# GDMCF/GDMCF

Measured on AMD Instinct MI355X. Metric: training users/sec, higher is better.
Workload: dtype f32; 1 GPU; yelp-shape synthetic rows, batch=400/GPU, dims=[1000], T=5, noise_scale=0.01, linear-var, mean_type=x0, reweight, AdamW lr=1e-5 (BASELINE configs[1]); n_items=34395, global_batch=400, parallelism=dp1, batch_rows=device CSR rows (CsrBatch)

## Files before the change

### gdmcf_amd/build.py

```python
import concurrent.futures
import hashlib
import os
import re
import subprocess
import sys

CSRC = os.path.join(os.path.dirname(os.path.abspath(__file__)), "csrc")
SOURCES = ["capi.hip", "dp_exchange.hip", "gemm_f32.hip", "gemm_bf16.hip", "gemm_split.hip", "gemm_small.hip", "gemm_dr.hip", "gemm_dr_tn.hip", "gemm_dr_fat.hip", "gemm_dr_kn.hip", "prep_input.hip", "noise.hip", "loss_tail.hip", "adamw.hip", "rows.hip", "reduce.hip", "linear.hip", "topk_spmm.hip", "spmm_bundle.hip", "score_topk.hip", "bpr.hip", "cat.hip", "gather_fwd.hip", "ntxent.hip", "latent_step.hip"]
HEADERS = ["common.h", "draws.h", "gemm_dr.h", "gemm_epilogue.h", os.path.join("..", "..", "include", "gdmcf_hip.h")]
LIB = os.path.join(CSRC, "libgdmcf_hip.so")
ASM_LINT = ("gemm_dr_tn.hip", "gemm_split.hip")
STORE_LINT = ("gemm_f32.hip", "gemm_bf16.hip", "gemm_dr_fat.hip", "gemm_dr_kn.hip", "score_topk.hip", "latent_step.hip")
NO_SPILL = ("gemm_f32.hip", "gemm_bf16.hip", "gemm_split.hip", "gemm_dr_tn.hip", "score_topk.hip", "cat.hip", "gather_fwd.hip", "ntxent.hip", "latent_step.hip")
FLAGS = ["--offload-arch=gfx950", "-O3", "-std=c++17", "-fPIC", "-Wall", "-Wno-unused-function"]


def _hipcc():
    for c in (os.environ.get("HIPCC"), "/opt/rocm/bin/hipcc", "hipcc"):
        if c and (os.path.isabs(c) and os.path.exists(c) or not os.path.isabs(c)):
            return c
    raise RuntimeError("hipcc not found")


def _digest():
    h = hashlib.sha256()
    for f in SOURCES + HEADERS:
        with open(os.path.join(CSRC, f), "rb") as fh:
            h.update(fh.read())
    h.update(" ".join(FLAGS).encode())
    return h.hexdigest()


_REG = re.compile(r"\bv(\d+)\b|\bv\[(\d+):(\d+)\]")


def _regs(text):
    out = set()
    for m in _REG.finditer(text):
        if m.group(1) is not None:
            out.add(int(m.group(1)))
        else:
            out.update(range(int(m.group(2)), int(m.group(3)) + 1))
    return out


_SREG = re.compile(r"\bs(\d+)\b|\bs\[(\d+):(\d+)\]")


def _sregs(text):
    out = set()
    for m in _SREG.finditer(text):
        if m.group(1) is not None:
            out.add(int(m.group(1)))
        else:
            out.update(range(int(m.group(2)), int(m.group(3)) + 1))
    return out


def lint_ring_registers(asm_text, kernel_prefix="dr_tn_kernel"):
    bad, seen = [], 0
    for m in re.finditer(r"^(\S*%s\S*):[^\n]*\n(.*?)\n\s*s_endpgm" % kernel_prefix, asm_text, flags=re.S | re.M):
        name, body = m.group(1), m.group(2)
        seen += 1
        lines = [ln.split(";")[0].strip() for ln in body.splitlines()]
        lines = [ln for ln in lines if ln and not ln.endswith(":") and not ln.startswith(".")]
        ring = set()
# ... 107 lines not shown

        state = [None] * len(blocks)
        state[0] = {}
        work = [0]
        while work:
            bi = work.pop()
            out = transfer(bi, state[bi], False)
            for sj in succ[bi]:
                if state[sj] is None:
                    state[sj] = dict(out)
                    work.append(sj)
                else:
                    changed = False
                    for r, rk in out.items():
                        if state[sj].get(r, 65) > rk:
                            state[sj][r] = rk
                            changed = True
                    if changed:
                        work.append(sj)
        for bi in range(len(blocks)):
            if state[bi] is not None:
                transfer(bi, state[bi], True)
        bad += [f"{name}: {msg}" for msg, k in sorted(found.items(), key=lambda kv: kv[1])]
    if not nk:
        bad.append("no kernel with inline-asm loads in the assembly (lint out of date?)")
    return bad


def lint_store_data(asm_text):
    bad = []
    for m in re.finditer(r"^(_Z\S+):[^\n]*\n(.*?)\n\s*s_endpgm", asm_text, flags=re.S | re.M):
        name, body = m.group(1), m.group(2)
        lines = [ln.split(";")[0].strip() for ln in body.splitlines()]
        lines = [ln for ln in lines if ln and not ln.startswith(".") and not ln.endswith(":")]
        for k, ln in enumerate(lines):
            mnem, _, ops = ln.partition(" ")
            if not re.match(r"(buffer|global|flat|scratch)_store_dwordx[34]$", mnem):
                continue
            parts = [o.strip() for o in ops.split(",")]
            data = _regs(parts[1] if mnem.startswith(("global", "flat", "scratch")) else parts[0])
            left = 2
            for nxt in lines[k + 1:k + 8]:
                nm, _, nops = nxt.partition(" ")
                if nm == "s_nop":
                    left -= int(nops.strip() or 0) + 1
                else:
                    nparts = [o.strip() for o in nops.split(",")]
                    if nm.startswith("v_") and nparts and _regs(nparts[0]) & data and left > 0:
                        bad.append(f"{name}: data register of `{ln}` rewritten {2 - left} wait state(s) later by `{nxt}`")
                        break
                    left -= 1
                if left <= 0:
                    break
    return bad


def build(force=False, verbose=True):
    stamp = os.path.join(CSRC, ".build_stamp")
    dig = _digest()
    if not force and os.path.exists(LIB) and os.path.exists(stamp) and open(stamp).read() == dig:
        return LIB
    hipcc = _hipcc()
    objs = []

    def compile_one(src):
        obj = os.path.join(CSRC, src.replace(".hip", ".o"))
        cmd = [hipcc] + FLAGS + ["-c", os.path.join(CSRC, src), "-o", obj]
        guarded = src in NO_SPILL
        if guarded:
            cmd.append("-Rpass-analysis=kernel-resource-usage")
        r = subprocess.run(cmd, capture_output=True, text=True)
        if r.returncode != 0:
            raise RuntimeError(f"hipcc failed for {src}:\n{r.stderr}")
        err = r.stderr
        if guarded:
            name, bad = None, []
            for line in err.splitlines():
                if "Function Name:" in line:
                    name = line.split("Function Name:")[1].split()[0]
                elif "VGPRs Spill:" in line and int(line.split("VGPRs Spill:")[1].split()[0]) > 0:
                    bad.append(name)
            if bad:
                raise RuntimeError(f"{src}: register spills in {len(bad)} kernel(s) with uncounted asm loads, e.g. {bad[0]}")
            err = err if ("warning:" in err or "error:" in err) else ""
        if verbose and err.strip():
            print(err, file=sys.stderr)
        if src in ASM_LINT or src in STORE_LINT:
            asm = os.path.join(CSRC, src.replace(".hip", ".lint.s"))
            r2 = subprocess.run([hipcc] + FLAGS + ["-S", "--cuda-device-only", os.path.join(CSRC, src), "-o", asm],
                                capture_output=True, text=True)
            if r2.returncode != 0:
                raise RuntimeError(f"hipcc -S failed for {src}:\n{r2.stderr}")
            text = open(asm).read()
            os.remove(asm)
            bad = lint_store_data(text)
            if src in ASM_LINT:
                bad += lint_vmcnt(text)
            if src == "gemm_dr_tn.hip":
                bad += lint_ring_registers(text)
            if bad:
                raise RuntimeError(f"{src}: ISA lint failed (lint_store_data / lint_vmcnt / lint_ring_registers):\n  " + "\n  ".join(bad[:12]))
        return obj

    with concurrent.futures.ThreadPoolExecutor(max_workers=min(8, len(SOURCES))) as ex:
        objs = list(ex.map(compile_one, SOURCES))
    cmd = [hipcc, "--offload-arch=gfx950", "-shared", "-fPIC", "-o", LIB] + objs
    r = subprocess.run(cmd, capture_output=True, text=True)
    if r.returncode != 0:
        raise RuntimeError(f"link failed:\n{r.stderr}")
    with open(stamp, "w") as fh:
        fh.write(dig)
    if verbose:
        print(f"built {LIB}")
    return LIB


if __name__ == "__main__":
    build(force="--force" in sys.argv)
```

### gdmcf_amd/csrc/gemm_dr.h

```cpp
#pragma once

#include "common.h"

namespace {
struct DrArgs {
    GdGemm g;
    int tiles_m, tiles_n, m_fastest;
    int ksp;
    int ctr;
    const GdAdamHyper* adam_dev;
    int stagger;
};
}

struct DrRoutes {
    bool dw;
    bool adamw;
    bool kn;
    bool fat;
};
DrRoutes& dr_routes();
int dr_cu_count();
int dr_stagger();

int gd_dr_tn_launch(GdGemm& g, hipStream_t s);
int gd_dr_kn_launch(GdGemm& g, hipStream_t s);
int gd_dr_fat_launch(int epi, GdGemm& g, hipStream_t s);
```

### gdmcf_amd/csrc/gemm_dr.hip

```cpp
#include <stdlib.h>

#include "gemm_dr.h"

int dr_cu_count() {
    static int n_cu = 0;
    if (n_cu == 0) {
        int dev = 0;
        hipDeviceProp_t prop;
        n_cu = (hipGetDevice(&dev) == hipSuccess && hipGetDeviceProperties(&prop, dev) == hipSuccess) ? prop.multiProcessorCount : 256;
    }
    return n_cu;
}

static bool dr_env_on(const char* name) {
    const char* v = getenv(name);
    return v == nullptr || atoi(v) != 0;
}
DrRoutes& dr_routes() {
    static DrRoutes r = {dr_env_on("GDMCF_DR_DW"), dr_env_on("GDMCF_DR_ADAMW"), dr_env_on("GDMCF_DR_KN"), dr_env_on("GDMCF_DR_FAT")};
    return r;
}

int dr_stagger() {
    static const int stagger = getenv("GDMCF_DR_STAGGER") ? atoi(getenv("GDMCF_DR_STAGGER")) : 3;
    return stagger;
}

int gd_gemm_dr_launch(int layA, int layB, int epi, GdGemm& g, hipStream_t s) {
    if (g.bf16) return GD_DR_NOT_TAKEN;
    if (g.accumulate || g.C16 || (g.splits > 1 && epi != GD_EPI_SLAB)) return GD_DR_NOT_TAKEN;
    if (layA == GD_LAY_MC && layB == GD_LAY_MC) {
        if (epi == GD_EPI_ADAMW) return gd_gemm_dr_adamw_multi(&g, 1, s);
        if (epi == GD_EPI_STORE) return gd_dr_tn_launch(g, s);
    } else if (layA == GD_LAY_KC && layB == GD_LAY_MC) {
        if (epi == GD_EPI_SLAB) return gd_dr_kn_launch(g, s);
    } else if (layA == GD_LAY_KC && layB == GD_LAY_KC) {
        if (epi == GD_EPI_LOSS || epi == GD_EPI_POST) return gd_dr_fat_launch(epi, g, s);
    }
    return GD_DR_NOT_TAKEN;
}
```

### gdmcf_amd/csrc/linear.hip

```cpp
#include <stdlib.h>

#include "common.h"

int gd_splitk_reduce(const float* slabs, int64_t slab_stride, int splits, int64_t ld_slab, int M, int N, int mode,
                     const float* bias, const float* rowscale, const float* aact, int64_t ldact, int act, float* out,
                     int64_t ldo, hipStream_t s);
int gd_colsum(const float* dZ, int64_t ld, const float* rs, int M, int N, float* db, hipStream_t s);
int gd_rowpart_reduce(const float* rowpart, int ld, int M, int nt, float* rowsum, hipStream_t s);

namespace {

static const int TARGET_WGS = getenv("GDMCF_TARGET_WGS") ? atoi(getenv("GDMCF_TARGET_WGS")) : 760;

thread_local int t_gemm_prec = GDMCF_GEMM_F32;

int pick_class(int M, int N, bool fused, int prec) {
    if (prec == GDMCF_GEMM_BF16 && M > 128) {
        const long pad = (long)gd_cdiv(M, 208) * 208;
        const long tiles = (pad / 208) * gd_cdiv(N, 256);
        const long rounds = (tiles + 255) / 256;
        if (pad * 10 <= (long)M * 11 && pad / 208 <= 2 && (!fused || tiles * 100 >= rounds * 256 * 85)) return 3;
    }
    if (prec == GDMCF_GEMM_F32X3 && M > 128 && N >= 128) {
        const long pad = (long)gd_cdiv(M, 208) * 208;
// ... 84 lines not shown
    const int prev = t_gemm_prec;
    if (mode == GDMCF_GEMM_F32 || mode == GDMCF_GEMM_BF16 || mode == GDMCF_GEMM_F32X3) t_gemm_prec = mode;
    return prev;
}

size_t gdmcf_linear_ws_bytes(int M, int N, int K) {
    if (M <= 0 || N <= 0 || K <= 0) return 0;
    size_t need = 0;
    for (int prec = GDMCF_GEMM_F32; prec <= GDMCF_GEMM_F32X3; ++prec) {
        const int cf = pick_class(M, N, false, prec), cb = pick_class(M, K, false, prec);
        size_t f = (size_t)pick_splits(M, N, K, cf, prec) * M * round4(N);
        if (prec == GDMCF_GEMM_F32) {
            const size_t fk = (size_t)gd_dr_kn_splits(M, N, K) * M * round4(N);
            f = f > fk ? f : fk;
        }
        size_t b = (size_t)pick_splits(M, K, N, cb, prec) * M * round4(K);
        if (prec == GDMCF_GEMM_F32) {
            const size_t bk = (size_t)gd_dr_kn_splits(M, K, N) * M * round4(K);
            b = b > bk ? b : bk;
        }
        need = need > f ? need : f;
        need = need > b ? need : b;
    }
    return need * sizeof(float) + 256;
}

int gdmcf_loss_tiles(int N) { return gd_cdiv(N, 16); }

int gdmcf_linear_fwd_f32(const float* A, int64_t lda, const float* W, int64_t ldw, const float* bias, int act, int M,
                         int N, int K, float* C, int64_t ldc, void* ws, size_t ws_bytes, void* stream) {
    GD_CHECK_SHAPE(M > 0 && N > 0 && K > 0 && lda >= K && ldw >= K && ldc >= N, "linear_fwd: bad shape");
    GD_CHECK_ARG(act == 0 || act == 1, "linear_fwd: bad activation");
    hipStream_t s = (hipStream_t)stream;
    const int cls = pick_class(M, N, false, t_gemm_prec);
    const int splits = pick_splits(M, N, K, cls, t_gemm_prec);
    GdGemm g = {};
    g.bf16 = t_gemm_prec;
    g.A = A; g.lda = lda; g.B = W; g.ldb = ldw; g.M = M; g.N = N; g.K = K;
    g.m_fastest = gd_cdiv(M, gd_gemm_tile_m(cls)) <= gd_cdiv(N, gd_gemm_tile_n(cls));
    g.bias = bias; g.act = act; g.prof_tag = 1;
    if (splits == 1) {
        g.splits = 1; g.C = C; g.ldc = ldc;
        attach_result_shadow(g);
        attach_shadows(g, GD_LAY_KC, GD_LAY_KC);
        return gd_gemm_launch(GD_LAY_KC, GD_LAY_KC, GD_EPI_BIAS_ACT, cls, g, s);
    }
    const int64_t lds_ = round4(N);
    const size_t need = (size_t)splits * M * lds_ * sizeof(float);
    if (ws == nullptr || ws_bytes < need) {
        gdmcf_set_error("linear_fwd: workspace %zu < %zu bytes", ws_bytes, need);
        return GDMCF_E_WORKSPACE;
    }
    g.splits = splits; g.C = (float*)ws; g.ldc = lds_; g.slab_stride = (int64_t)M * lds_;
    attach_shadows(g, GD_LAY_KC, GD_LAY_KC);
    int rc = gd_gemm_launch(GD_LAY_KC, GD_LAY_KC, GD_EPI_SLAB, cls, g, s);
    if (rc) return rc;
    const int real_splits = gd_cdiv(K, g.kchunk);
    return gd_splitk_reduce((const float*)ws, g.slab_stride, real_splits, lds_, M, N, 0, bias, nullptr, nullptr, 0,
                            act, C, ldc, s);
}

int gdmcf_linear_fwd_wt_f32(const float* A, int64_t lda, const float* Wt, int64_t ldwt, const float* bias, int act, int M, int N,
                            int K, float* C, int64_t ldc, void* ws, size_t ws_bytes, void* stream) {
    GD_CHECK_SHAPE(M > 0 && N > 0 && K > 0 && lda >= K && ldwt >= N && ldc >= N, "linear_fwd_wt: bad shape");
    GD_CHECK_ARG(act == 0 || act == 1, "linear_fwd_wt: bad activation");
    if (t_gemm_prec != GDMCF_GEMM_F32) {
        gdmcf_set_error("linear_fwd_wt: float32 GEMM mode only (the bf16 / f32x3 modes keep the weight in its own orientation)");
        return GDMCF_E_UNSUPPORTED;
    }
    hipStream_t s = (hipStream_t)stream;
    const int cls = pick_class(M, N, false, t_gemm_prec);
    const int splits = pick_splits(M, N, K, cls, t_gemm_prec);
    const int64_t lds_ = round4(N);
    const size_t need = (size_t)splits * M * lds_ * sizeof(float);
    if (ws == nullptr || ws_bytes < need) {
        gdmcf_set_error("linear_fwd_wt: workspace %zu < %zu bytes", ws_bytes, need);
        return GDMCF_E_WORKSPACE;
    }
    GdGemm g = {};
    g.A = A; g.lda = lda; g.B = Wt; g.ldb = ldwt; g.M = M; g.N = N; g.K = K;
    g.m_fastest = gd_cdiv(M, gd_gemm_tile_m(cls)) <= gd_cdiv(N, gd_gemm_tile_n(cls));
    g.splits = splits; g.C = (float*)ws; g.ldc = lds_; g.slab_stride = (int64_t)M * lds_; g.prof_tag = 1;
    g.ws_cap = ws_bytes;
    int rc = gd_gemm_launch(GD_LAY_KC, GD_LAY_MC, GD_EPI_SLAB, cls, g, s);
    if (rc) return rc;
    const int real_splits = gd_cdiv(K, g.kchunk);
    return gd_splitk_reduce((const float*)ws, g.slab_stride, real_splits, lds_, M, N, 0, bias, nullptr, nullptr, 0, act, C, ldc, s);
}

int gdmcf_linear_loss_fwd_f32(const float* A, int64_t lda, const float* W, int64_t ldw, const float* bias,
                              const float* target, int64_t ldt, const float* alpha, int M, int N, int K, float* out,
                              int64_t ldo, float* diff, int64_t ldd, float* rowpart, float* rowsum, void* stream) {
    GD_CHECK_SHAPE(M > 0 && N > 0 && K > 0 && lda >= K && ldw >= K && ldt >= N && ldd >= N, "linear_loss_fwd: bad shape");
    GD_CHECK_SHAPE(out == nullptr || ldo >= N, "linear_loss_fwd: ldo < N");
    hipStream_t s = (hipStream_t)stream;
    const int cls = pick_class(M, N, true, t_gemm_prec);
    GdGemm g = {};
    g.bf16 = t_gemm_prec;
    g.A = A; g.lda = lda; g.B = W; g.ldb = ldw; g.M = M; g.N = N; g.K = K; g.splits = 1;
    g.m_fastest = gd_cdiv(M, gd_gemm_tile_m(cls)) <= gd_cdiv(N, gd_gemm_tile_n(cls));
    g.bias = bias; g.aux = target; g.ldaux = ldt; g.r0 = alpha; g.out2 = out; g.ldout2 = ldo;
    g.prof_tag = 2;
    g.C = diff; g.ldc = ldd; g.rowpart = rowpart; g.ld_rowpart = gdmcf_loss_tiles(N);
    attach_result_shadow(g);
    attach_shadows(g, GD_LAY_KC, GD_LAY_KC);
    int rc = gd_gemm_launch(GD_LAY_KC, GD_LAY_KC, GD_EPI_LOSS, cls, g, s);
// ... 150 lines not shown
```

### gdmcf_amd/csrc/gemm_dr_fat.hip

```cpp
#include <stdlib.h>

#include "gemm_dr.h"

namespace {

template <int NB, int EPI>
__global__ __launch_bounds__(256, 1) void dr_fat_kernel(const DrArgs d) {
    static_assert(EPI == GD_EPI_LOSS || EPI == GD_EPI_POST, "output layer with a fused epilogue");
    static_assert(NB >= 4 && NB <= 12, "5 x NB accumulator blocks must fit 256 registers");
    constexpr int TMB = 5;
    const GdGemm& g = d.g;
    const int lane = threadIdx.x & 63;
    const int wave = __builtin_amdgcn_readfirstlane(threadIdx.x >> 6);
    const int r = lane & 15, q = lane >> 4;
    extern __shared__ __attribute__((aligned(16))) float dr_lds[];
    float* const lds = dr_lds + wave * (2 * NB * 256);
    const int nblk = gridDim.x, per = nblk >> 3;
    const int wl = ((nblk & 7) == 0 ? ((int)(blockIdx.x & 7) * per + (int)(blockIdx.x >> 3)) : (int)blockIdx.x) * 4 + wave;
    const int n_waves = nblk * 4;
    const int ntiles = d.tiles_m * d.tiles_n;
    const __amdgpu_buffer_rsrc_t srdA = __builtin_amdgcn_make_buffer_rsrc(const_cast<float*>(g.A), 0, (int)(((int64_t)(g.M - 1) * g.lda + g.K) * 4), 0x00020000);
    const __amdgpu_buffer_rsrc_t srdB = __builtin_amdgcn_make_buffer_rsrc(const_cast<float*>(g.B), 0, (int)(((int64_t)(g.N - 1) * g.ldb + g.K) * 4), 0x00020000);
    const int NCH = d.ksp;
    const int c_mask = g.K >> 4;
    const int w_off = (lane >> 2) * 16 + (((lane & 3) ^ ((((lane >> 2) >> 2) & 1) << 1)) << 2);
    const int r_off = r * 16 + ((q ^ (((r >> 2) & 1) << 1)) << 2);
    for (int tile = wl; tile < ntiles; tile += n_waves) {
        const int tm = tile % d.tiles_m, tn = tile / d.tiles_m;
        const int m0 = tm * (16 * TMB), n0 = tn * (16 * NB);
        uint32_t offA[TMB], offB[NB];
#pragma unroll
        for (int i = 0; i < TMB; ++i) offA[i] = (uint32_t)((m0 + 16 * i + r) * g.lda + 4 * q) * 4u;
#pragma unroll
        for (int p = 0; p < NB; ++p) offB[p] = (uint32_t)(((int64_t)(n0 + 16 * p + (lane >> 2)) * g.ldb + 4 * (lane & 3)) * 4);
        f32x4 acc[TMB][NB];
#pragma unroll
        for (int i = 0; i < TMB; ++i)
#pragma unroll
            for (int b = 0; b < NB; ++b) acc[i][b] = f32x4{0.f, 0.f, 0.f, 0.f};
        f32x4 xa[2][TMB], G[NB], FB[NB];
#pragma unroll
        for (int i = 0; i < TMB; ++i) xa[0][i] = __builtin_bit_cast(f32x4, __builtin_amdgcn_raw_buffer_load_b128(srdA, offA[i], 0, 0));
#pragma unroll
        for (int p = 0; p < NB; ++p) G[p] = __builtin_bit_cast(f32x4, __builtin_amdgcn_raw_buffer_load_b128(srdB, offB[p], 0, 0));
#pragma unroll
        for (int p = 0; p < NB; ++p) *reinterpret_cast<f32x4*>(lds + p * 256 + w_off) = G[p];

#define GD_FAT_CHUNK(PAR, c)                                                                                          \
        {                                                                                                             \
             \
            const uint32_t kn = ((c) + 1 < NCH) ? (uint32_t)((c) + 1) * 64u : 0x80000000u;                            \
            _Pragma("unroll") for (int b = 0; b < NB; ++b)                                                            \
                FB[b] = *reinterpret_cast<const f32x4*>(lds + (PAR) * (NB * 256) + b * 256 + r_off);                  \
            if ((c) >= c_mask) {  \
                 \
                _Pragma("unroll") for (int e = 0; e < 4; ++e) {                                                       \
                    const bool keep = (c) * 16 + 4 * q + e < g.K;                                                     \
                    _Pragma("unroll") for (int i = 0; i < TMB; ++i) xa[PAR][i][e] = keep ? xa[PAR][i][e] : 0.f;       \
                    _Pragma("unroll") for (int b = 0; b < NB; ++b) FB[b][e] = keep ? FB[b][e] : 0.f;                  \
                }                                                                                                     \
            }                                                                                                         \
            __builtin_amdgcn_sched_barrier(0);                                                                        \
            _Pragma("unroll") for (int sx = 0; sx < 4; ++sx) {                                                        \
                _Pragma("unroll") for (int n = 0; n < TMB * NB; ++n) {                                                \
                    const int i = n / NB, b = n % NB;                                                                 \
                    if (sx == 0 && i == 0) asm volatile("" : "+v"(FB[b]));  \
                    if (sx == 0 && b == 0) asm volatile("" : "+v"(xa[PAR][i]));                                       \
                    acc[i][b] = __builtin_amdgcn_mfma_f32_16x16x4f32(xa[PAR][i][sx], FB[b][sx], acc[i][b], 0, 0, 0);  \
                     \
                    if (sx < 2 && n % 5 == 2) {      \
                        const int l = (sx == 0) ? n / 5 : NB + n / 5;                                                 \
                        if (l < TMB + NB) {                                                                           \
                            __builtin_amdgcn_sched_barrier(0);                                                        \
                            if (l < TMB)                                                                              \
                                xa[(PAR) ^ 1][l] = __builtin_bit_cast(f32x4, __builtin_amdgcn_raw_buffer_load_b128(   \
                                    srdA, offA[l], kn, 0));                                                           \
                            else                                                                                      \
                                G[l - TMB] = __builtin_bit_cast(f32x4, __builtin_amdgcn_raw_buffer_load_b128(         \
                                    srdB, offB[l - TMB], kn, 0));                                                     \
                            __builtin_amdgcn_sched_barrier(0);                                                        \
                        }                                                                                             \
                    }                                                                                                 \
                    if (sx == 3 && n % 4 == 1 && n / 4 < NB) {   \
                        __builtin_amdgcn_sched_barrier(0);                                                            \
                        *reinterpret_cast<f32x4*>(lds + ((PAR) ^ 1) * (NB * 256) + (n / 4) * 256 + w_off) = G[n / 4]; \
                        __builtin_amdgcn_sched_barrier(0);                                                            \
                    }                                                                                                 \
                }                                                                                                     \
                __builtin_amdgcn_sched_barrier(0);                                                                    \
            }                                                                                                         \
        }
        const int c_pf = d.stagger > 0 ? ((NCH > d.stagger + 2 ? NCH - d.stagger : 0) & ~1) : -2;
        for (int c = 0; c + 1 < NCH; c += 2) {
            if constexpr (EPI == GD_EPI_POST) {
                if (c == c_pf) {
                    typedef __attribute__((address_space(3))) void* lds_vp;
                    constexpr int NJL = (16 * NB * 4 + 127) / 128 + 1;
                    constexpr int NPI = (80 * NJL + 63) / 64;
                    float* const scratch = dr_lds + 4 * (2 * NB * 256) + wave * 64;
                    const __amdgpu_buffer_rsrc_t srdX = __builtin_amdgcn_make_buffer_rsrc(
                        const_cast<float*>(g.aux), 0, (int)(((int64_t)(g.M - 1) * g.ldaux + g.N) * 4), 0x00020000);
#pragma unroll
                    for (int pi = 0; pi < NPI; ++pi) {
                        const int t = min(pi * 64 + lane, 80 * NJL - 1);
                        const int row = min(m0 + t % 80, g.M - 1), j = t / 80;
                        const int col = min(j < NJL - 1 ? n0 + 32 * j : n0 + 16 * NB - 1, g.N - 1);
                        __builtin_amdgcn_raw_ptr_buffer_load_lds(srdX, (lds_vp)scratch, 4, (int)(((int64_t)row * g.ldaux + col) * 4), 0, 0, 0);
                    }
                }
            }
            GD_FAT_CHUNK(0, c);
            GD_FAT_CHUNK(1, c + 1);
        }
        if (NCH & 1) GD_FAT_CHUNK(0, NCH - 1);
#undef GD_FAT_CHUNK

        constexpr int LDS_ = 16 * NB + 4;
        constexpr int NJ = (4 * NB + 15) / 16;
        typedef f32x4 f32x4_e __attribute__((aligned(4)));
        f32x4 bias4[NJ];
        int col4[NJ];
#pragma unroll
        for (int j = 0; j < NJ; ++j) {
            col4[j] = n0 + 4 * (r + 16 * j);
            bias4[j] = f32x4{0.f, 0.f, 0.f, 0.f};
            if (g.bias && r + 16 * j < 4 * NB) {
#pragma unroll
                for (int e = 0; e < 4; ++e) bias4[j][e] = g.bias[min(col4[j] + e, g.N - 1)];
            }
        }
        const bool has_z = (EPI == GD_EPI_POST) && (g.aux2 != nullptr);
        const bool has_r = (EPI == GD_EPI_POST) && (g.r2 != nullptr);
        struct Pre {
            f32x4 a[NJ], z[NJ];
            uint32_t w[NJ];
            float c1, c2, p1, p2, sg;
        } pre[2];
        auto fetch = [&](int i, int p4, Pre& P) {
            const int mc = min(m0 + 16 * i + 4 * p4 + q, g.M - 1);
            P.c1 = 1.f; P.c2 = 0.f; P.p1 = 0.f; P.p2 = 0.f; P.sg = 0.f;
            if (EPI == GD_EPI_LOSS) {
                if (g.r0) P.c1 = g.r0[mc];
            } else {
                P.c1 = g.r0[mc];
                P.c2 = g.r1[mc];
                if (has_r) { P.p1 = g.r2[mc]; P.p2 = g.r3[mc]; }
                if (has_z) P.sg = g.r4[mc];
            }
#pragma unroll
            for (int j = 0; j < NJ; ++j) {
                const int n = col4[j];
                const bool whole = (r + 16 * j < 4 * NB) && n + 3 < g.N;
                P.w[j] = 0u;
                P.a[j] = f32x4{0.f, 0.f, 0.f, 0.f};
                P.z[j] = f32x4{0.f, 0.f, 0.f, 0.f};
                if (EPI == GD_EPI_LOSS && g.aux_bits) {
                    P.w[j] = g.aux_bits[(int64_t)mc * g.ldbits + min((int64_t)(n >> 5), g.ldbits - 1)];
                } else if (whole) {
                    P.a[j] = *reinterpret_cast<const f32x4_e*>(g.aux + (int64_t)mc * g.ldaux + n);
                    if (has_z) P.z[j] = *reinterpret_cast<const f32x4_e*>(g.aux2 + (int64_t)mc * g.ldaux2 + n);
                }
            }
        };
        fetch(0, 0, pre[0]);
#pragma unroll
        for (int i = 0; i < TMB; ++i) {
#pragma unroll
            for (int b = 0; b < NB; ++b)
// ... 28 lines not shown
                        } else if (whole) {
                            tg = P.a[j];
                        } else {
#pragma unroll
                            for (int e = 0; e < 4; ++e) tg[e] = g.aux[(int64_t)mc * g.ldaux + min(n + e, g.N - 1)];
                        }
#pragma unroll
                        for (int e = 0; e < 4; ++e) {
                            o2[e] = v[e] + bias4[j][e];
                            o[e] = c1 * o2[e] - tg[e];
                            if (inb && mok && n + e < g.N) ss += o[e] * o[e];
                        }
                    } else {
                        f32x4 xt = P.a[j], zz = P.z[j];
                        if (!whole) {
#pragma unroll
                            for (int e = 0; e < 4; ++e) {
                                xt[e] = g.aux[(int64_t)mc * g.ldaux + min(n + e, g.N - 1)];
                                if (has_z) zz[e] = g.aux2[(int64_t)mc * g.ldaux2 + min(n + e, g.N - 1)];
                            }
                        }
#pragma unroll
                        for (int e = 0; e < 4; ++e) {
                            const float vv = v[e] + bias4[j][e];
                            o2[e] = has_r ? (p1 * xt[e] - p2 * vv) : vv;
                            o[e] = c1 * o2[e] + c2 * xt[e];
                            if (has_z) o[e] += sg * zz[e];
                        }
                    }
                    if (full) {
                        *reinterpret_cast<f32x4_e*>(g.C + (int64_t)m * g.ldc + n) = o;
                        if (g.out2) *reinterpret_cast<f32x4_e*>(g.out2 + (int64_t)m * g.ldout2 + n) = o2;
                    } else if (inb && mok) {
                        for (int e = 0; e < 4 && n + e < g.N; ++e) {
                            g.C[(int64_t)m * g.ldc + n + e] = o[e];
                            if (g.out2) g.out2[(int64_t)m * g.ldout2 + n + e] = o2[e];
                        }
                    }
                }
                if (EPI == GD_EPI_LOSS) {
                    ss += __shfl_xor(ss, 1);
                    ss += __shfl_xor(ss, 2);
                    ss += __shfl_xor(ss, 4);
                    ss += __shfl_xor(ss, 8);
                    if (r == 0 && mok) g.rowpart[(int64_t)m * g.ld_rowpart + tn] = ss;
                }
                __builtin_amdgcn_sched_barrier(0);
            }
        }
    }
}

template <int NB>
int dr_fat_go(const DrArgs& d, int epi, int n_cu, hipStream_t s) {
    const size_t lds = (size_t)4 * 2 * NB * 256 * sizeof(float) + 4 * 64 * sizeof(float);
    void (*kern)(const DrArgs) = epi == GD_EPI_LOSS ? dr_fat_kernel<NB, GD_EPI_LOSS> : dr_fat_kernel<NB, GD_EPI_POST>;
    static bool attr_set[2] = {false, false};
    if (!attr_set[epi == GD_EPI_LOSS] && lds > 48 * 1024) {
        hipError_t e = hipFuncSetAttribute(reinterpret_cast<const void*>(kern), hipFuncAttributeMaxDynamicSharedMemorySize, (int)lds);
        if (e != hipSuccess) {
            gdmcf_set_error("hipFuncSetAttribute(dr_fat_kernel, LDS=%zu): %s", lds, hipGetErrorString(e));
            return GDMCF_E_HIP;
        }
        attr_set[epi == GD_EPI_LOSS] = true;
    }
    hipLaunchKernelGGL(kern, dim3(n_cu), dim3(256), lds, s, d);
    return GDMCF_OK;
}

}

int gd_dr_fat_launch(int epi, GdGemm& g, hipStream_t s) {
    if (!dr_routes().fat) return GD_DR_NOT_TAKEN;
    const int64_t lim = (int64_t)1 << 32;
    const int n_cu = dr_cu_count();
    const int tiles_m = gd_cdiv(g.M, 80);
    bool ok = (int64_t)g.M * g.lda * 4 < ((int64_t)1 << 31) && (int64_t)g.N * g.ldb * 4 < lim && g.lda >= g.K && g.ldb >= g.K &&
              g.K >= 256 && (long)tiles_m * 80 * 100 <= (long)g.M * 112 &&
              (n_cu & 7) == 0 && !(epi == GD_EPI_LOSS && g.rowpart == nullptr) &&
              !(epi == GD_EPI_LOSS && g.aux_bits && g.ldbits < (g.N + 31) / 32);
    int nb = 0;
    long best = 1L << 60;
    const long slots = 4L * n_cu;
    for (int c = 12; c >= 8 && ok; --c) {
        const long t = (long)tiles_m * gd_cdiv(g.N, 16 * c);
        const long cost = ((t + slots - 1) / slots) * c;
        if (t >= slots / 2 && cost < best) { best = cost; nb = c; }
    }
    if (ok && epi == GD_EPI_POST) {
        const long t128 = (long)gd_cdiv(g.M, 80) * gd_cdiv(g.N, 128);
        const long rounds = (t128 + 2 * n_cu - 1) / (2 * n_cu);
        if (t128 * 100 >= rounds * 2 * n_cu * 90) ok = false;
    }
    if (!ok || !nb || (epi == GD_EPI_LOSS && g.ld_rowpart < gd_cdiv(g.N, 16 * nb))) return GD_DR_NOT_TAKEN;
    DrArgs d = {};
    d.tiles_m = tiles_m;
    d.tiles_n = gd_cdiv(g.N, 16 * nb);
    d.m_fastest = 1;
    d.ksp = gd_cdiv(g.K, 16);
    {
        static const int pf = getenv("GDMCF_FAT_PF") ? atoi(getenv("GDMCF_FAT_PF")) : 10;
        d.stagger = pf;
    }
    g.tiles_m = d.tiles_m;
    g.tiles_n = d.tiles_n;
    d.g = g;
    d.ctr = 0;
    int rc = GDMCF_OK;
    {
        GdProfScope prof(g.prof_tag, 2.0 * g.M * g.N * g.K, s);
        switch (nb) {
            case 8: rc = dr_fat_go<8>(d, epi, n_cu, s); break;
            case 9: rc = dr_fat_go<9>(d, epi, n_cu, s); break;
            case 10: rc = dr_fat_go<10>(d, epi, n_cu, s); break;
            case 11: rc = dr_fat_go<11>(d, epi, n_cu, s); break;
            default: rc = dr_fat_go<12>(d, epi, n_cu, s); break;
        }
    }
    if (rc != GDMCF_OK) return rc;
    t_gd_last_gemm = 4;
    return gd_launch_status("gemm_dr");
}
```

Before: 312,500 users/s.

## Add direct-register split-K GEMM kernel for KC x KC slab linear forward

Adds a new persistent split-K f32 MFMA kernel for the linear forward GEMM with both operands K-contiguous and slab output. It loads operands straight from global memory into registers with buffer loads, double-buffers them and interleaves the next chunk's loads between MFMAs under scheduling barriers. Each wave owns an 80x128 tile and bypasses LDS. The aim is to cut LDS traffic and synchronisation in the existing generic path, at the cost of heavy register pressure and reliance on the split count chosen by the kn heuristic.

```diff
diff --git a/gdmcf_amd/build.py b/gdmcf_amd/build.py
--- a/gdmcf_amd/build.py
+++ b/gdmcf_amd/build.py
@@ -6,12 +6,12 @@
 import sys
 
 CSRC = os.path.join(os.path.dirname(os.path.abspath(__file__)), "csrc")
-SOURCES = ["capi.hip", "dp_exchange.hip", "gemm_f32.hip", "gemm_bf16.hip", "gemm_split.hip", "gemm_small.hip", "gemm_dr.hip", "gemm_dr_tn.hip", "gemm_dr_fat.hip", "gemm_dr_kn.hip", "prep_input.hip", "noise.hip", "loss_tail.hip", "adamw.hip", "rows.hip", "reduce.hip", "linear.hip", "topk_spmm.hip", "spmm_bundle.hip", "score_topk.hip", "bpr.hip", "cat.hip", "gather_fwd.hip", "ntxent.hip", "latent_step.hip"]
+SOURCES = ["capi.hip", "dp_exchange.hip", "gemm_f32.hip", "gemm_bf16.hip", "gemm_split.hip", "gemm_small.hip", "gemm_dr.hip", "gemm_dr_tn.hip", "gemm_dr_fat.hip", "gemm_dr_kn.hip", "gemm_dr_kk.hip", "prep_input.hip", "noise.hip", "loss_tail.hip", "adamw.hip", "rows.hip", "reduce.hip", "linear.hip", "topk_spmm.hip", "spmm_bundle.hip", "score_topk.hip", "bpr.hip", "cat.hip", "gather_fwd.hip", "ntxent.hip", "latent_step.hip"]
 HEADERS = ["common.h", "draws.h", "gemm_dr.h", "gemm_epilogue.h", os.path.join("..", "..", "include", "gdmcf_hip.h")]
 LIB = os.path.join(CSRC, "libgdmcf_hip.so")
 ASM_LINT = ("gemm_dr_tn.hip", "gemm_split.hip")
-STORE_LINT = ("gemm_f32.hip", "gemm_bf16.hip", "gemm_dr_fat.hip", "gemm_dr_kn.hip", "score_topk.hip", "latent_step.hip")
-NO_SPILL = ("gemm_f32.hip", "gemm_bf16.hip", "gemm_split.hip", "gemm_dr_tn.hip", "score_topk.hip", "cat.hip", "gather_fwd.hip", "ntxent.hip", "latent_step.hip")
+STORE_LINT = ("gemm_f32.hip", "gemm_bf16.hip", "gemm_dr_fat.hip", "gemm_dr_kn.hip", "gemm_dr_kk.hip", "score_topk.hip", "latent_step.hip")
+NO_SPILL = ("gemm_f32.hip", "gemm_bf16.hip", "gemm_split.hip", "gemm_dr_tn.hip", "score_topk.hip", "cat.hip", "gather_fwd.hip", "ntxent.hip", "latent_step.hip", "gemm_dr_kk.hip")
 FLAGS = ["--offload-arch=gfx950", "-O3", "-std=c++17", "-fPIC", "-Wall", "-Wno-unused-function"]
 
 
diff --git a/gdmcf_amd/csrc/gemm_dr.h b/gdmcf_amd/csrc/gemm_dr.h
--- a/gdmcf_amd/csrc/gemm_dr.h
+++ b/gdmcf_amd/csrc/gemm_dr.h
@@ -18,6 +18,7 @@
     bool adamw;
     bool kn;
     bool fat;
+    bool kk;
 };
 DrRoutes& dr_routes();
 int dr_cu_count();
@@ -26,3 +27,4 @@
 int gd_dr_tn_launch(GdGemm& g, hipStream_t s);
 int gd_dr_kn_launch(GdGemm& g, hipStream_t s);
 int gd_dr_fat_launch(int epi, GdGemm& g, hipStream_t s);
+int gd_dr_kk_launch(GdGemm& g, hipStream_t s);
diff --git a/gdmcf_amd/csrc/gemm_dr.hip b/gdmcf_amd/csrc/gemm_dr.hip
--- a/gdmcf_amd/csrc/gemm_dr.hip
+++ b/gdmcf_amd/csrc/gemm_dr.hip
@@ -17,7 +17,8 @@
     return v == nullptr || atoi(v) != 0;
 }
 DrRoutes& dr_routes() {
-    static DrRoutes r = {dr_env_on("GDMCF_DR_DW"), dr_env_on("GDMCF_DR_ADAMW"), dr_env_on("GDMCF_DR_KN"), dr_env_on("GDMCF_DR_FAT")};
+    static DrRoutes r = {dr_env_on("GDMCF_DR_DW"), dr_env_on("GDMCF_DR_ADAMW"), dr_env_on("GDMCF_DR_KN"), dr_env_on("GDMCF_DR_FAT"),
+                       dr_env_on("GDMCF_DR_KK")};
     return r;
 }
 
@@ -36,6 +37,7 @@
         if (epi == GD_EPI_SLAB) return gd_dr_kn_launch(g, s);
     } else if (layA == GD_LAY_KC && layB == GD_LAY_KC) {
         if (epi == GD_EPI_LOSS || epi == GD_EPI_POST) return gd_dr_fat_launch(epi, g, s);
+        if (epi == GD_EPI_SLAB) return gd_dr_kk_launch(g, s);
     }
     return GD_DR_NOT_TAKEN;
 }
diff --git a/gdmcf_amd/csrc/gemm_dr_kk.hip b/gdmcf_amd/csrc/gemm_dr_kk.hip
--- /dev/null
+++ b/gdmcf_amd/csrc/gemm_dr_kk.hip
@@ -0,0 +1,129 @@
+#include "gemm_dr.h"
+
+namespace {
+
+#ifndef GD_KK_EVERY
+#define GD_KK_EVERY 4
+#endif
+__global__ __launch_bounds__(256, 1) void dr_kk_kernel(const DrArgs d) {
+    constexpr int TMB = 5, TNB = 8;
+    const GdGemm& g = d.g;
+    const int lane = threadIdx.x & 63;
+    const int wave = __builtin_amdgcn_readfirstlane(threadIdx.x >> 6);
+    const int r = lane & 15, q = lane >> 4;
+    const int nblk = gridDim.x, per = nblk >> 3;
+    const int wl = ((nblk & 7) == 0 ? ((int)(blockIdx.x & 7) * per + (int)(blockIdx.x >> 3)) : (int)blockIdx.x) * 4 + wave;
+    const int n_waves = nblk * 4;
+    const int ntiles = d.tiles_m * d.tiles_n;
+    const int CPS = d.ksp;
+    const int total_chunks = (g.K + 15) >> 4;
+    const int ntasks = ntiles * g.splits;
+    const __amdgpu_buffer_rsrc_t srdA = __builtin_amdgcn_make_buffer_rsrc(const_cast<float*>(g.A), 0, (int)(((int64_t)(g.M - 1) * g.lda + g.K) * 4), 0x00020000);
+    const __amdgpu_buffer_rsrc_t srdB = __builtin_amdgcn_make_buffer_rsrc(const_cast<float*>(g.B), 0, (int)(((int64_t)(g.N - 1) * g.ldb + g.K) * 4), 0x00020000);
+    for (int task = wl; task < ntasks; task += n_waves) {
+        const int split = task / ntiles, tile = task - split * ntiles;
+        const int tm = tile % d.tiles_m, tn = tile / d.tiles_m;
+        const int m0 = tm * (16 * TMB), n0 = tn * (16 * TNB);
+        const int c_lo = split * CPS;
+        uint32_t offA[TMB], offB[TNB];
+#pragma unroll
+        for (int a = 0; a < TMB; ++a) offA[a] = (uint32_t)(((int64_t)min(m0 + 16 * a + r, g.M - 1) * g.lda + 4 * q) * 4);
+#pragma unroll
+        for (int b = 0; b < TNB; ++b) {
+            const int n = n0 + 16 * b + r;
+            offB[b] = n < g.N ? (uint32_t)(((int64_t)n * g.ldb + 4 * q) * 4) : 0x80000000u;
+        }
+        f32x4 acc[TMB][TNB];
+#pragma unroll
+        for (int a = 0; a < TMB; ++a)
+#pragma unroll
+            for (int b = 0; b < TNB; ++b) acc[a][b] = f32x4{0.f, 0.f, 0.f, 0.f};
+        f32x4 xa[2][TMB], xb[2][TNB];
+        {
+            const uint32_t kk = (uint32_t)c_lo * 64u;
+#pragma unroll
+            for (int a = 0; a < TMB; ++a) xa[0][a] = __builtin_bit_cast(f32x4, __builtin_amdgcn_raw_buffer_load_b128(srdA, offA[a], kk, 0));
+#pragma unroll
+            for (int b = 0; b < TNB; ++b) xb[0][b] = __builtin_bit_cast(f32x4, __builtin_amdgcn_raw_buffer_load_b128(srdB, offB[b], kk, 0));
+        }
+#define GD_KK_CHUNK(PAR, c)                                                                                            \
+        {                                                                                                              \
+            const bool more = (c) + 1 < c_lo + CPS && (c) + 1 < total_chunks;                                          \
+            const uint32_t kk = more ? (uint32_t)((c) + 1) * 64u : 0x80000000u;                                        \
+            if ((c) * 16 + 15 >= g.K) {          \
+                _Pragma("unroll") for (int e = 0; e < 4; ++e) {                                                        \
+                    const bool keep = (c) * 16 + 4 * q + e < g.K;                                                      \
+                    _Pragma("unroll") for (int a = 0; a < TMB; ++a) xa[PAR][a][e] = keep ? xa[PAR][a][e] : 0.f;        \
+                    _Pragma("unroll") for (int b = 0; b < TNB; ++b) xb[PAR][b][e] = keep ? xb[PAR][b][e] : 0.f;        \
+                }                                                                                                      \
+            }                                                                                                          \
+                    \
+            _Pragma("unroll") for (int a = 0; a < TMB; ++a) asm volatile("" : "+v"(xa[PAR][a]));                       \
+            _Pragma("unroll") for (int b = 0; b < TNB; ++b) asm volatile("" : "+v"(xb[PAR][b]));                       \
+            __builtin_amdgcn_sched_barrier(0);                                                                         \
+            _Pragma("unroll") for (int s = 0; s < 4; ++s) {                                                            \
+                _Pragma("unroll") for (int n = 0; n < TMB * TNB; ++n) {                                                \
+                    const int a = n / TNB, b = n % TNB;                                                                \
+                    acc[a][b] = __builtin_amdgcn_mfma_f32_16x16x4f32(xb[PAR][b][s], xa[PAR][a][s], acc[a][b], 0, 0, 0); \
+                    const int idx = s * (TMB * TNB) + n;                                                               \
+                    if (idx % GD_KK_EVERY == 2 && idx / GD_KK_EVERY < TMB + TNB) {                                     \
+                        const int ld = idx / GD_KK_EVERY;                                                              \
+                        __builtin_amdgcn_sched_barrier(0);                                                             \
+                        if (ld < TMB)                                                                                  \
+                            xa[(PAR) ^ 1][ld] = __builtin_bit_cast(f32x4, __builtin_amdgcn_raw_buffer_load_b128(srdA, offA[ld], kk, 0)); \
+                        else                                                                                           \
+                            xb[(PAR) ^ 1][ld - TMB] = __builtin_bit_cast(f32x4, __builtin_amdgcn_raw_buffer_load_b128(srdB, offB[ld - TMB], kk, 0)); \
+                        __builtin_amdgcn_sched_barrier(0);                                                             \
+                    }                                                                                                  \
+                }                                                                                                      \
+                __builtin_amdgcn_sched_barrier(0);                                                                     \
+            }                                                                                                          \
+        }
+        for (int c = c_lo; c < c_lo + CPS && c < total_chunks; c += 2) {
+            GD_KK_CHUNK(0, c);
+            GD_KK_CHUNK(1, c + 1);
+        }
+#undef GD_KK_CHUNK
+        float* __restrict__ slab = g.C + (int64_t)split * g.slab_stride;
+#pragma unroll
+        for (int a = 0; a < TMB; ++a) {
+            const int m = m0 + 16 * a + r;
+#pragma unroll
+            for (int b = 0; b < TNB; ++b) {
+                const int n = n0 + 16 * b + 4 * q;
+                if (m < g.M && n < g.ldc) *reinterpret_cast<f32x4*>(slab + (int64_t)m * g.ldc + n) = acc[a][b];
+            }
+        }
+    }
+}
+
+}
+
+int gd_dr_kk_launch(GdGemm& g, hipStream_t s) {
+    if (!dr_routes().kk) return GD_DR_NOT_TAKEN;
+    const int splits = gd_dr_kn_splits(g.M, g.N, g.K);
+    const size_t need = (size_t)splits * (size_t)g.slab_stride * sizeof(float);    const int64_t lim = (int64_t)1 << 31;
+    const bool ok = splits > 0 && g.ldc >= g.N && (g.ldc & 3) == 0 && g.ws_cap >= need && g.slab_stride >= (int64_t)g.M * g.ldc &&
+                    (int64_t)g.M * g.lda * 4 < lim && (int64_t)g.N * g.ldb * 4 < lim && g.lda >= g.K && g.ldb >= g.K &&
+                    (reinterpret_cast<uintptr_t>(g.A) & 3) == 0 && (reinterpret_cast<uintptr_t>(g.B) & 3) == 0 &&
+                    (reinterpret_cast<uintptr_t>(g.C) & 15) == 0 && (g.slab_stride & 3) == 0;
+    if (!ok) return GD_DR_NOT_TAKEN;
+    DrArgs d = {};
+    const int n_cu = dr_cu_count();
+    const int total_chunks = gd_cdiv(g.K, 16);
+    const int cps = (gd_cdiv(total_chunks, splits) + 1) & ~1;
+    d.tiles_m = gd_cdiv(g.M, 80);
+    d.tiles_n = gd_cdiv(g.N, 128);
+    d.ksp = cps;
+    g.splits = gd_cdiv(total_chunks, cps);
+    g.kchunk = cps * 16;
+    g.tiles_m = d.tiles_m;
+    g.tiles_n = d.tiles_n;
+    d.g = g;
+    {
+        GdProfScope prof(g.prof_tag, 2.0 * g.M * g.N * g.K, s);
+        hipLaunchKernelGGL(dr_kk_kernel, dim3(n_cu), dim3(256), 0, s, d);
+    }
+    t_gd_last_gemm = 10;
+    return gd_launch_status("gemm_dr_kk");
+}
diff --git a/gdmcf_amd/csrc/linear.hip b/gdmcf_amd/csrc/linear.hip
--- a/gdmcf_amd/csrc/linear.hip
+++ b/gdmcf_amd/csrc/linear.hip
@@ -160,6 +160,7 @@
         return GDMCF_E_WORKSPACE;
     }
     g.splits = splits; g.C = (float*)ws; g.ldc = lds_; g.slab_stride = (int64_t)M * lds_;
+    g.ws_cap = ws_bytes;
     attach_shadows(g, GD_LAY_KC, GD_LAY_KC);
     int rc = gd_gemm_launch(GD_LAY_KC, GD_LAY_KC, GD_EPI_SLAB, cls, g, s);
     if (rc) return rc;
```

New measurement: 314,500 users/s, median of 6. About the same (+0.6%).

## Load fat-GEMM B tiles straight into LDS with buffer_load_lds DMA

Applied to the files above, without the earlier changes.

Adds a DMA variant of the fat output-layer GEMM kernel that loads B chunks directly into LDS via buffer_load ... lds, instead of staging them through registers and writing them with ds_write. This is meant to cut VGPR pressure and LDS store instructions in the k loop. The price is a full vmcnt(0) wait before each chunk's LDS reads, which may expose load latency, plus a parity-shifted chunk schedule and reworked K-tail masking. A build-time ISA lint checks the wait ordering and that the k loop has no spills, and the path is enabled by default when B is 16-byte aligned.

```diff
diff --git a/gdmcf_amd/build.py b/gdmcf_amd/build.py
--- a/gdmcf_amd/build.py
+++ b/gdmcf_amd/build.py
@@ -225,6 +225,43 @@
                     left -= 1
                 if left <= 0:
                     break
+    return bad
+
+
+def lint_fat_dma(asm_text, kernel="dr_fat_kernel"):
+    bad, n_dma = [], 0
+    for m in re.finditer(r"^(_Z\S*%s\S*):[^\n]*\n(.*?)\n\s*s_endpgm" % kernel, asm_text, flags=re.S | re.M):
+        name, body = m.group(1), m.group(2)
+        lines = [ln.split(";")[0].strip() for ln in body.splitlines()]
+        lines = [ln for ln in lines if ln and (not ln.startswith(".") or ln.endswith(":"))]
+        if not any(ln.startswith("buffer_load_dwordx4") and ln.endswith(" lds") for ln in lines):
+            continue
+        n_dma += 1
+        pending = None
+        for ln in lines:
+            if ln.startswith("buffer_load_dwordx4") and ln.endswith(" lds"):
+                pending = ln
+            elif ln.startswith("s_waitcnt") and re.search(r"vmcnt\(0\)", ln):
+                pending = None
+            elif ln.startswith("ds_read_b128") and pending:
+                bad.append(f"{name}: `{ln}` follows `{pending}` with no s_waitcnt vmcnt(0) in between")
+                break
+        loops, label, blk = 0, None, []
+        for ln in lines + ["end:"]:
+            if not ln.endswith(":"):
+                blk.append(ln)
+                continue
+            if label and any(i.startswith("v_mfma") for i in blk) and any(
+                    i.startswith(("s_cbranch", "s_branch")) and i.split()[-1] == label for i in blk):
+                loops += 1
+                moved = [i for i in blk if i.startswith(("scratch_", "v_accvgpr", "v_mov"))]
+                if moved:
+                    bad.append(f"{name}: {len(moved)} spill / move instruction(s) in the k loop, e.g. `{moved[0]}`")
+            label, blk = ln[:-1], []
+        if not loops:
+            bad.append(f"{name}: no k loop found (lint out of date?)")
+    if not n_dma:
+        bad.append(f"no *{kernel}* with `buffer_load_dwordx4 ... lds` in the assembly (lint out of date?)")
     return bad
 
 
@@ -271,8 +308,10 @@
                 bad += lint_vmcnt(text)
             if src == "gemm_dr_tn.hip":
                 bad += lint_ring_registers(text)
+            if src == "gemm_dr_fat.hip":
+                bad += lint_fat_dma(text)
             if bad:
-                raise RuntimeError(f"{src}: ISA lint failed (lint_store_data / lint_vmcnt / lint_ring_registers):\n  " + "\n  ".join(bad[:12]))
+                raise RuntimeError(f"{src}: ISA lint failed (lint_store_data / lint_vmcnt / lint_ring_registers / lint_fat_dma):\n  " + "\n  ".join(bad[:12]))
         return obj
 
     with concurrent.futures.ThreadPoolExecutor(max_workers=min(8, len(SOURCES))) as ex:
diff --git a/gdmcf_amd/csrc/gemm_dr_fat.hip b/gdmcf_amd/csrc/gemm_dr_fat.hip
--- a/gdmcf_amd/csrc/gemm_dr_fat.hip
+++ b/gdmcf_amd/csrc/gemm_dr_fat.hip
@@ -2,12 +2,19 @@
 
 #include "gemm_dr.h"
 
+#ifndef GD_FAT_DMA_DEFAULT
+#define GD_FAT_DMA_DEFAULT 1
+#endif
+
 namespace {
 
-template <int NB, int EPI>
+template <int NB, int EPI, int DMA>
 __global__ __launch_bounds__(256, 1) void dr_fat_kernel(const DrArgs d) {
     static_assert(EPI == GD_EPI_LOSS || EPI == GD_EPI_POST, "output layer with a fused epilogue");
     static_assert(NB >= 4 && NB <= 12, "5 x NB accumulator blocks must fit 256 registers");
+    static_assert(DMA == 0 || DMA == 1, "B through staging registers, or straight into LDS");
+    typedef __attribute__((address_space(3))) void* lds_vp;
+    constexpr int WAIT_VM0 = 0x0F70, WAIT_LGKM0 = 0xC07F;
     constexpr int TMB = 5;
     const GdGemm& g = d.g;
     const int lane = threadIdx.x & 63;
@@ -24,6 +31,7 @@
     const int NCH = d.ksp;
     const int c_mask = g.K >> 4;
     const int w_off = (lane >> 2) * 16 + (((lane & 3) ^ ((((lane >> 2) >> 2) & 1) << 1)) << 2);
+    const int g_slot = DMA ? ((lane & 3) ^ ((((lane >> 2) >> 2) & 1) << 1)) : (lane & 3);
     const int r_off = r * 16 + ((q ^ (((r >> 2) & 1) << 1)) << 2);
     for (int tile = wl; tile < ntiles; tile += n_waves) {
         const int tm = tile % d.tiles_m, tn = tile / d.tiles_m;
@@ -32,27 +40,46 @@
 #pragma unroll
         for (int i = 0; i < TMB; ++i) offA[i] = (uint32_t)((m0 + 16 * i + r) * g.lda + 4 * q) * 4u;
 #pragma unroll
-        for (int p = 0; p < NB; ++p) offB[p] = (uint32_t)(((int64_t)(n0 + 16 * p + (lane >> 2)) * g.ldb + 4 * (lane & 3)) * 4);
+        for (int p = 0; p < NB; ++p) offB[p] = (uint32_t)(((int64_t)(n0 + 16 * p + (lane >> 2)) * g.ldb + 4 * g_slot) * 4);
         f32x4 acc[TMB][NB];
 #pragma unroll
         for (int i = 0; i < TMB; ++i)
 #pragma unroll
             for (int b = 0; b < NB; ++b) acc[i][b] = f32x4{0.f, 0.f, 0.f, 0.f};
-        f32x4 xa[2][TMB], G[NB], FB[NB];
-#pragma unroll
-        for (int i = 0; i < TMB; ++i) xa[0][i] = __builtin_bit_cast(f32x4, __builtin_amdgcn_raw_buffer_load_b128(srdA, offA[i], 0, 0));
-#pragma unroll
-        for (int p = 0; p < NB; ++p) G[p] = __builtin_bit_cast(f32x4, __builtin_amdgcn_raw_buffer_load_b128(srdB, offB[p], 0, 0));
-#pragma unroll
-        for (int p = 0; p < NB; ++p) *reinterpret_cast<f32x4*>(lds + p * 256 + w_off) = G[p];
-
-#define GD_FAT_CHUNK(PAR, c)                                                                                          \
+        f32x4 xa[2][TMB], G[DMA ? 1 : NB], FB[NB];
+        const int hp = DMA ? (c_mask & 1) : 0;
+        if (hp) {
+#pragma unroll
+            for (int i = 0; i < TMB; ++i) xa[1][i] = __builtin_bit_cast(f32x4, __builtin_amdgcn_raw_buffer_load_b128(srdA, offA[i], 0, 0));
+        } else {
+#pragma unroll
+            for (int i = 0; i < TMB; ++i) xa[0][i] = __builtin_bit_cast(f32x4, __builtin_amdgcn_raw_buffer_load_b128(srdA, offA[i], 0, 0));
+        }
+        if constexpr (DMA) {
+            __builtin_amdgcn_sched_barrier(0);
+            __builtin_amdgcn_s_waitcnt(WAIT_LGKM0);
+            __builtin_amdgcn_sched_barrier(0);
+#pragma unroll
+            for (int p = 0; p < NB; ++p) __builtin_amdgcn_raw_ptr_buffer_load_lds(srdB, (lds_vp)(lds + hp * (NB * 256) + p * 256), 16, (int)offB[p], 0, 0, 0);
+        } else {
+#pragma unroll
+            for (int p = 0; p < NB; ++p) G[p] = __builtin_bit_cast(f32x4, __builtin_amdgcn_raw_buffer_load_b128(srdB, offB[p], 0, 0));
+#pragma unroll
+            for (int p = 0; p < NB; ++p) *reinterpret_cast<f32x4*>(lds + p * 256 + w_off) = G[p];
+        }
+
+#define GD_FAT_CHUNK(PAR, c, MSK)                                                                                         \
         {                                                                                                             \
              \
             const uint32_t kn = ((c) + 1 < NCH) ? (uint32_t)((c) + 1) * 64u : 0x80000000u;                            \
+            if constexpr (DMA) {                                                                                      \
+                __builtin_amdgcn_sched_barrier(0);                                                                    \
+                __builtin_amdgcn_s_waitcnt(WAIT_VM0);                                                                 \
+                __builtin_amdgcn_sched_barrier(0);                                                                    \
+            }                                                                                                         \
             _Pragma("unroll") for (int b = 0; b < NB; ++b)                                                            \
                 FB[b] = *reinterpret_cast<const f32x4*>(lds + (PAR) * (NB * 256) + b * 256 + r_off);                  \
-            if ((c) >= c_mask) {  \
+            if (MSK) {  \
                  \
                 _Pragma("unroll") for (int e = 0; e < 4; ++e) {                                                       \
                     const bool keep = (c) * 16 + 4 * q + e < g.K;                                                     \
@@ -75,13 +102,17 @@
                             if (l < TMB)                                                                              \
                                 xa[(PAR) ^ 1][l] = __builtin_bit_cast(f32x4, __builtin_amdgcn_raw_buffer_load_b128(   \
                                     srdA, offA[l], kn, 0));                                                           \
+                            else if constexpr (DMA)                                                                   \
+                                __builtin_amdgcn_raw_ptr_buffer_load_lds(                                             \
+                                    srdB, (lds_vp)(lds + ((PAR) ^ 1) * (NB * 256) + (l - TMB) * 256), 16,             \
+                                    (int)offB[l - TMB], (int)kn, 0, 0);                                               \
                             else                                                                                      \
                                 G[l - TMB] = __builtin_bit_cast(f32x4, __builtin_amdgcn_raw_buffer_load_b128(         \
                                     srdB, offB[l - TMB], kn, 0));                                                     \
                             __builtin_amdgcn_sched_barrier(0);                                                        \
                         }                                                                                             \
                     }                                                                                                 \
-                    if (sx == 3 && n % 4 == 1 && n / 4 < NB) {   \
+                    if (!DMA && sx == 3 && n % 4 == 1 && n / 4 < NB) {  \
                         __builtin_amdgcn_sched_barrier(0);                                                            \
                         *reinterpret_cast<f32x4*>(lds + ((PAR) ^ 1) * (NB * 256) + (n / 4) * 256 + w_off) = G[n / 4]; \
                         __builtin_amdgcn_sched_barrier(0);                                                            \
@@ -91,10 +122,18 @@
             }                                                                                                         \
         }
         const int c_pf = d.stagger > 0 ? ((NCH > d.stagger + 2 ? NCH - d.stagger : 0) & ~1) : -2;
-        for (int c = 0; c + 1 < NCH; c += 2) {
+        const int c_pairs = DMA ? c_mask : NCH;
+        const int c_pfl = (DMA && c_pf >= 0) ? min(c_pf | hp, c_pairs - 2) : c_pf;
+        int c = 0;
+        if constexpr (DMA) {
+            if (hp) {
+                GD_FAT_CHUNK(1, 0, false);
+                c = 1;
+            }
+        }
+        for (; c + 1 < c_pairs; c += 2) {
             if constexpr (EPI == GD_EPI_POST) {
-                if (c == c_pf) {
-                    typedef __attribute__((address_space(3))) void* lds_vp;
+                if (c == c_pfl) {
                     constexpr int NJL = (16 * NB * 4 + 127) / 128 + 1;
                     constexpr int NPI = (80 * NJL + 63) / 64;
                     float* const scratch = dr_lds + 4 * (2 * NB * 256) + wave * 64;
@@ -109,11 +148,25 @@
                     }
                 }
             }
-            GD_FAT_CHUNK(0, c);
-            GD_FAT_CHUNK(1, c + 1);
-        }
-        if (NCH & 1) GD_FAT_CHUNK(0, NCH - 1);
+            if constexpr (DMA) {
+                GD_FAT_CHUNK(0, c, false);
+                GD_FAT_CHUNK(1, c + 1, false);
+            } else {
+                GD_FAT_CHUNK(0, c, c >= c_mask);
+                GD_FAT_CHUNK(1, c + 1, c + 1 >= c_mask);
+            }
+        }
+        if constexpr (DMA) {
+            if (c < NCH) GD_FAT_CHUNK(0, c, true);
+        } else {
+            if (NCH & 1) GD_FAT_CHUNK(0, NCH - 1, NCH - 1 >= c_mask);
+        }
 #undef GD_FAT_CHUNK
+        if constexpr (DMA) {
+            __builtin_amdgcn_sched_barrier(0);
+            __builtin_amdgcn_s_waitcnt(WAIT_VM0);
+            __builtin_amdgcn_sched_barrier(0);
+        }
 
         constexpr int LDS_ = 16 * NB + 4;
         constexpr int NJ = (4 * NB + 15) / 16;
@@ -248,17 +301,19 @@
 }
 
 template <int NB>
-int dr_fat_go(const DrArgs& d, int epi, int n_cu, hipStream_t s) {
+int dr_fat_go(const DrArgs& d, int epi, int dma, int n_cu, hipStream_t s) {
     const size_t lds = (size_t)4 * 2 * NB * 256 * sizeof(float) + 4 * 64 * sizeof(float);
-    void (*kern)(const DrArgs) = epi == GD_EPI_LOSS ? dr_fat_kernel<NB, GD_EPI_LOSS> : dr_fat_kernel<NB, GD_EPI_POST>;
-    static bool attr_set[2] = {false, false};
-    if (!attr_set[epi == GD_EPI_LOSS] && lds > 48 * 1024) {
+    void (*kern)(const DrArgs) = dma ? (epi == GD_EPI_LOSS ? dr_fat_kernel<NB, GD_EPI_LOSS, 1> : dr_fat_kernel<NB, GD_EPI_POST, 1>)
+                                     : (epi == GD_EPI_LOSS ? dr_fat_kernel<NB, GD_EPI_LOSS, 0> : dr_fat_kernel<NB, GD_EPI_POST, 0>);
+    static bool attr_set[4] = {false, false, false, false};
+    const int ai = 2 * dma + (epi == GD_EPI_LOSS);
+    if (!attr_set[ai] && lds > 48 * 1024) {
         hipError_t e = hipFuncSetAttribute(reinterpret_cast<const void*>(kern), hipFuncAttributeMaxDynamicSharedMemorySize, (int)lds);
         if (e != hipSuccess) {
             gdmcf_set_error("hipFuncSetAttribute(dr_fat_kernel, LDS=%zu): %s", lds, hipGetErrorString(e));
             return GDMCF_E_HIP;
         }
-        attr_set[epi == GD_EPI_LOSS] = true;
+        attr_set[ai] = true;
     }
     hipLaunchKernelGGL(kern, dim3(n_cu), dim3(256), lds, s, d);
     return GDMCF_OK;
@@ -298,6 +353,8 @@
         static const int pf = getenv("GDMCF_FAT_PF") ? atoi(getenv("GDMCF_FAT_PF")) : 10;
         d.stagger = pf;
     }
+    static const int dma_env = getenv("GDMCF_FAT_DMA") ? atoi(getenv("GDMCF_FAT_DMA")) : GD_FAT_DMA_DEFAULT;
+    const int dma = (dma_env > 0 && (reinterpret_cast<uintptr_t>(g.B) & 15) == 0 && (g.ldb & 3) == 0) ? 1 : 0;
     g.tiles_m = d.tiles_m;
     g.tiles_n = d.tiles_n;
     d.g = g;
@@ -306,11 +363,11 @@
     {
         GdProfScope prof(g.prof_tag, 2.0 * g.M * g.N * g.K, s);
         switch (nb) {
-            case 8: rc = dr_fat_go<8>(d, epi, n_cu, s); break;
-            case 9: rc = dr_fat_go<9>(d, epi, n_cu, s); break;
-            case 10: rc = dr_fat_go<10>(d, epi, n_cu, s); break;
-            case 11: rc = dr_fat_go<11>(d, epi, n_cu, s); break;
-            default: rc = dr_fat_go<12>(d, epi, n_cu, s); break;
+            case 8: rc = dr_fat_go<8>(d, epi, dma, n_cu, s); break;
+            case 9: rc = dr_fat_go<9>(d, epi, dma, n_cu, s); break;
+            case 10: rc = dr_fat_go<10>(d, epi, dma, n_cu, s); break;
+            case 11: rc = dr_fat_go<11>(d, epi, dma, n_cu, s); break;
+            default: rc = dr_fat_go<12>(d, epi, dma, n_cu, s); break;
         }
     }
     if (rc != GDMCF_OK) return rc;
```

Measured after the change: 315,400 users/s before, 319,300 users/s after, median of 6. +1.2%, better.
